# juansgomez87/consensus-entropy

Measured on AMD Instinct MI355X. Metric: pool items scored+ranked/sec (M=16,C=4) at 1/2/4/8 GPUs; % HBM roofline, higher is better.
Workload: dtype f64; 1 GPU; configs[3] large-ensemble pool: 100000000 items x 16 members x 4 classes fp32, [N,M,C] layout=NMC, q=10, sharded over 1 GPU(s); n_items=100000000, members=16, classes=4, q=10, input_dtype=f32, layout=NMC, items_per_gpu=100000000

## Files before the change

### consensus-entropy_amd/csrc/ce_launch_stream.hip

```cpp
#include <atomic>

#include "ce_dispatch.hpp"
#include "ce_stream.hpp"
#include "ce_wide_stream.hpp"

using namespace ce;

static inline StreamArgs stream_args(const CommArgs& a, int G, int64_t base_idx) {
    StreamArgs s;
    s.p = a.p;
    s.N = a.N;
    s.M = a.M;
    s.sN = a.sN;
    s.sM = a.sM;
    s.sC = a.sC;
    s.dM = (double)a.M;
    s.invM = 1.0 / (double)a.M;
    s.pow2 = (a.M & (a.M - 1)) == 0;
    s.base_idx = base_idx;
    s.nlists = G;
    s.per_wave = 0;
    s.excl = nullptr;
    s.ctr = nullptr;
    s.oval = nullptr;
    s.oidx = nullptr;
    s.ocand = nullptr;
    s.extra = nullptr;
    s.vote = nullptr;
    s.vote_heavy = 0;
    s.seed = nullptr;
    s.claim = nullptr;
    s.claim_from = 0;
    return s;
}

static inline void stream_grid(StreamArgs& s, int grid) {
    const int64_t W = (int64_t)grid * 4;
    s.per_wave = (cdiv(s.N, W) + 63) / 64 * 64;
}

template <class Src, class F>
static inline void with_batching(int M, F&& f) {
    if constexpr (Src::kDT == kF64 || Src::kC > 4) {
        (void)M;
        f(std::integral_constant<int, 4>(), std::integral_constant<int, 2>());
    } else {
        if (M <= 4) f(std::integral_constant<int, 4>(), std::integral_constant<int, 4>());
        else f(std::integral_constant<int, 8>(), std::integral_constant<int, 2>());
    }
}


template <int UNR, class F>
static inline void with_unr(int unr, F&& f) {
    if (unr == UNR) f(std::integral_constant<int, UNR>());
    else f(std::integral_constant<int, 1>());
}

static int launch_stream_impl(const CommArgs& a, int G, int q, int64_t base_idx, WsLists w, hipStream_t st,
                              const uint32_t* excl, const FoldOut* fold);

#ifndef CE_STREAM_CLAIM_PERMILLE
#define CE_STREAM_CLAIM_PERMILLE 150
#endif
#ifndef CE_STREAM_CLAIM_MIN_ROUNDS
#define CE_STREAM_CLAIM_MIN_ROUNDS 300
#endif
static std::atomic<int64_t> g_claim_permille{-1}, g_claim_min_rounds{-1}, g_claim_from_last{0};
extern "C" void ce_debug_stream_claims(int64_t permille, int64_t min_rounds) {
    g_claim_permille = permille;
    g_claim_min_rounds = min_rounds;
}
extern "C" int64_t ce_debug_stream_claim_from() { return g_claim_from_last; }

static inline int64_t claim_from(int64_t N, int grid) {
    int64_t permille = g_claim_permille, min_rounds = g_claim_min_rounds;
    if (permille < 0) permille = CE_STREAM_CLAIM_PERMILLE;
    if (min_rounds < 0) min_rounds = CE_STREAM_CLAIM_MIN_ROUNDS;
    if (permille > 1000) permille = 1000;
    const int64_t rounds = cdiv(N, 64) / ((int64_t)grid * 4);
    if (rounds < min_rounds || permille == 0) return 0;
    const int64_t r = rounds - cdiv(rounds * permille, 1000);
    return r < 4 ? 4 : r;
}

#ifndef CE_NMC_AUX
#define CE_NMC_AUX 2
#endif

constexpr int64_t kWideHeavyBytes = 16384;

bool launch_stream(const CommArgs& a, int G, int q, int64_t base_idx, WsLists w, hipStream_t st,
                   const uint32_t* excl) {
    return launch_stream_impl(a, G, q, base_idx, w, st, excl, nullptr) != 0;
}

Stage1 launch_stream_fold(const CommArgs& a, int G, int q, int64_t base_idx, WsLists w, hipStream_t st,
                          const uint32_t* excl, FoldOut out) {
    return static_cast<Stage1>(launch_stream_impl(a, G, q, base_idx, w, st, excl, &out));
}

static int launch_stream_impl(const CommArgs& a, int G, int q, int64_t base_idx, WsLists w, hipStream_t st,
                              const uint32_t* excl, const FoldOut* fold) {
    note_kernel("%s", "");
    if (q > kStreamMaxQ || a.N == 0) return 0;
    StreamArgs sa = stream_args(a, G, base_idx);
    sa.excl = excl;
    if (fold) {
        sa.ctr = w.ctr;
        sa.oval = fold->oval;
        sa.oidx = fold->oidx;
        sa.ocand = fold->ocand;
        sa.extra = fold->extra;
    }
    const int folded = fold ? 2 : 1;
    const int eb = elem_bytes(a.dt);
    const int64_t R = (int64_t)a.M * a.C * eb;
    const bool dense_nmc = a.sC == 1 && a.sM == a.C && a.sN == (int64_t)a.M * a.C && (uintptr_t)a.p % 16 == 0;
#define CE_NMC(MATCH_, DT_, C_, S_, AUX_, MNC_)                                                             \
    if (a.dt == DT_ && a.C == C_ && (MATCH_)) {                                                           \
                   \
        constexpr int RING_ = S_ == 16 ? 2 : 1;                                                           \
        auto kern = k_stream_nmc<DT_, C_, S_, AUX_, MNC_, RING_>;                                         \
        const int grid = resident_grid(kern, 0, G);                                                       \
        note_kernel("ce::k_stream_nmc<%d, %d, %d, %d, %s, %d>", DT_, C_, S_, AUX_, MNC_ ? "true" : "false", \
                    RING_);                                                                               \
        stream_grid(sa, grid);                                                                            \
        g_claim_from_last = 0;                                                                            \
        if (fold && !MNC_ && RING_ == 2 && DT_ == kF32 && C_ == 4 && CE_STREAM_CLAIM_K > 0) {             \
            sa.claim_from = claim_from(a.N, grid);                    \
            sa.claim = sa.claim_from > 0 ? w.ctr + kWsClaimSlot : nullptr;                                \
            g_claim_from_last = sa.claim_from;                                                            \
        }                                                                                                 \
        hipLaunchKernelGGL(kern, dim3(grid), dim3(256), 0, st, sa, q, w.c);                               \
        return folded;                                                                                    \
    }
    if (dense_nmc && (R == 256 || R == 512)) {
#define CE_S(DT_, C_, S_) CE_NMC(R == 16 * S_, DT_, C_, S_, CE_NMC_AUX, false)
        CE_S(kF32, 4, 16) CE_S(kF32, 4, 32) CE_S(kBF16, 4, 16) CE_S(kBF16, 4, 32) CE_S(kF64, 4, 32)
        CE_S(kF32, 8, 16) CE_S(kF32, 8, 32)
#undef CE_S
    }
    const bool dense_mnc = a.sC == 1 && a.sN == a.C && a.C * eb == 16 && (a.sM * eb) % 16 == 0 &&
                           (uintptr_t)a.p % 16 == 0 && a.M >= 4;
    if (dense_mnc) {
#define CE_SM(DT_, C_, M_) CE_NMC(a.M == M_, DT_, C_, M_, 2, true)
        CE_SM(kF32, 4, 4) CE_SM(kF32, 4, 8) CE_SM(kF32, 4, 16) CE_SM(kF32, 4, 20) CE_SM(kF32, 4, 32)
        CE_SM(kF64, 2, 8) CE_SM(kF64, 2, 16) CE_SM(kBF16, 8, 16)
#undef CE_SM
    }
#undef CE_NMC
    int rc = with_committee(a, [&](auto src) {
        using S = decltype(src);
        with_batching<S>(a.M, [&](auto unr, auto ipl) {
            auto kern = k_stream_direct<S, decltype(ipl)::value, decltype(unr)::value>;
            note_kernel("ce::k_stream_direct<ce::CommitteeSrc<%d, %d, %s>, %d, %d>", S::kDT, S::kC,
                        S::kVec ? "true" : "false", decltype(ipl)::value, decltype(unr)::value);
            const int grid = resident_grid(kern, 0, G);
            stream_grid(sa, grid);
            hipLaunchKernelGGL(kern, dim3(grid), dim3(256), 0, st, src, sa, q, w.c);
        });
    });
    if (rc == CE_OK) return folded;
    if (a.C > kWideMaxC) return 0;
    const WideArgs wa = wide_args(a);
    const PwPlan pl = pw_plan(a.C);
    const size_t lds = wide_lds_bytes(a.C);
    int rc_excl = CE_OK;
    bool wide_folded = fold != nullptr;
    rc = with_wide_v(a, [&](auto dt, auto npl, auto vec) {
        constexpr int DT = decltype(dt)::value, NPL = decltype(npl)::value;
        if constexpr (decltype(vec)::value) {
            constexpr int KCH = NPL / ChunkT<DT>::CPC > 0 ? NPL / ChunkT<DT>::CPC : 1;
            constexpr int UNR = KCH >= 4 ? 1 : 4 / KCH;
            const int unr = a.M % UNR == 0 ? UNR : 1;
            auto go = [&](auto kern, int nb, int per_cu, StreamArgs s) {
                note_kernel("ce::k_stream_wide2<%d, %d, %d, %d>", DT, KCH, unr, nb);
                const int grid = std::min(resident_grid(kern, lds, G), per_cu * device_cus());
                stream_grid(s, grid);
                hipLaunchKernelGGL(kern, dim3(grid), dim3(256), lds, st, wa, pl, s, q, w.c);
            };
            bool voted = false;
            if constexpr (KCH <= 2)
                voted = R >= kWideHeavyBytes && fold != nullptr && fold->wide_ws != nullptr &&
                        a.N >= kWideSeedMinItems && CE_WIDE_PREFILTER;
            if (voted) {
                if constexpr (KCH <= 2) {
                    const WideSeedWs sw = wide_seed_carve(fold->wide_ws);
                    const int ns = (int)wide_nsamples(a.N);
                    with_unr<UNR>(unr, [&](auto u) {
                        hipLaunchKernelGGL((k_wide_seed<DT, KCH, decltype(u)::value>), dim3((unsigned)cdiv(ns, 4)),
                                           dim3(256), lds, st, wa, pl, sa.base_idx, sa.excl, sw.samp, sw.sapx);
                    });
                    hipLaunchKernelGGL(k_wide_seed_pick<kWideVoteSamples>, dim3(1), dim3(1024), 0, st, sw.samp, sw.sapx, ns, q,
                                       fold->extra, sw.seed, sw.vote);
                    StreamArgs sh = sa, so = sa;
                    sh.vote = so.vote = sw.vote;
                    sh.seed = so.seed = sw.seed;
                    sh.vote_heavy = 1;
                    so.vote_heavy = 0;
                    with_unr<UNR>(unr, [&](auto u) {
                        go(k_stream_wide2<DT, KCH, decltype(u)::value, 8>, 8, 1, sh);
                        go(k_stream_wide2<DT, KCH, decltype(u)::value, 2>, 2, 1 << 20, so);
                    });
                    note_kernel("ce::k_stream_wide2<%d, %d, %d, 8>|ce::k_stream_wide2<%d, %d, %d, 2>", DT, KCH, unr,
                                DT, KCH, unr);
                }
            } else {
                with_unr<UNR>(unr, [&](auto u) { go(k_stream_wide2<DT, KCH, decltype(u)::value, 2>, 2, 1 << 20, sa); });
            }
        } else {
            if (sa.excl) {
                rc_excl = CE_EUNSUPPORTED;
                return;
            }
            sa.ctr = nullptr;
            wide_folded = false;
            auto kern = k_stream_wide<DT, NPL, false>;
            note_kernel("ce::k_stream_wide<%d, %d, false>", DT, NPL);
            const int grid = resident_grid(kern, lds, G);
            stream_grid(sa, grid);
            hipLaunchKernelGGL(kern, dim3(grid), dim3(256), lds, st, wa, pl, sa, q, w.c);
        }
    });
    if (rc != CE_OK || rc_excl != CE_OK) return 0;
    return wide_folded ? 2 : 1;
}

#ifdef CE_STREAM_STAMPS
extern "C" int ce_debug_stream_stamps(uint64_t* host, int waves) {
    if (waves < 0 || waves > kStampWaves) return -1;
    return hipMemcpyFromSymbol(host, HIP_SYMBOL(g_stream_stamps), (size_t)waves * kStampCols * sizeof(uint64_t)) ==
                   hipSuccess
               ? 0
               : -1;
}
extern "C" int ce_debug_stream_stamp_cols() { return kStampCols; }
#endif
```

### consensus-entropy_amd/csrc/ce_stream.hpp

```cpp
#pragma once
#include "ce_device.hpp"
#include "ce_merge.hpp"
#include "ce_topq.hpp"
#include "ce_wave.hpp"
#include "ce_ws.hpp"

namespace ce {

template <int S>
struct ItemTile {
    uint32_t u[S * 4];

    template <int AUX>
    __device__ __forceinline__ static void issue(const char* base, int64_t t0, int n_valid, char* lds) {
        const int lane = threadIdx.x & 63;
#pragma unroll
        for (int k = 0; k < S; ++k) {
            const int p = k * 64 + lane;
            const int r = p / S, s = p % S;
            const int rs = r < n_valid ? r : n_valid - 1;
            const int m = s ^ (r & 15);
            const char* src = base + (t0 + rs) * (int64_t)(16 * S) + 16 * m;
            __builtin_amdgcn_global_load_lds(
                (const void*)src, (void __attribute__((address_space(3)))*)(lds + k * 1024), 16, 0, AUX);
        }
    }

    template <int AUX>
    __device__ __forceinline__ static void issue_mnc(const char* base, int64_t t0, int n_valid, int64_t sMb,
                                                     char* lds) {
        const int lane = threadIdx.x & 63;
        const int64_t it = t0 + (lane < n_valid ? lane : n_valid - 1);
#pragma unroll
        for (int k = 0; k < S; ++k) {
            const char* src = base + (int64_t)k * sMb + it * 16;
            __builtin_amdgcn_global_load_lds(
                (const void*)src, (void __attribute__((address_space(3)))*)(lds + k * 1024), 16, 0, AUX);
        }
    }

    __device__ __forceinline__ void read_mnc(const char* lds) {
        const int lane = threadIdx.x & 63;
        typedef unsigned int u32x4 __attribute__((ext_vector_type(4)));
#pragma unroll
        for (int m = 0; m < S; ++m) {
            const u32x4 v = *reinterpret_cast<const u32x4*>(lds + m * 1024 + lane * 16);
            u[4 * m + 0] = v.x;
            u[4 * m + 1] = v.y;
            u[4 * m + 2] = v.z;
            u[4 * m + 3] = v.w;
        }
    }

    __device__ __forceinline__ void read(const char* lds) {
        const int lane = threadIdx.x & 63;
        typedef unsigned int u32x4 __attribute__((ext_vector_type(4)));
#pragma unroll
        for (int m = 0; m < S; ++m) {
            const u32x4 v = *reinterpret_cast<const u32x4*>(lds + lane * 16 * S + 16 * (m ^ (lane & 15)));
            u[4 * m + 0] = v.x;
            u[4 * m + 1] = v.y;
            u[4 * m + 2] = v.z;
            u[4 * m + 3] = v.w;
        }
    }

    template <int DT>
    __device__ __forceinline__ double elem(int e) const {
        if constexpr (DT == kF32)
            return (double)__uint_as_float(u[e]);
        else if constexpr (DT == kF64)
            return __longlong_as_double((long long)(((uint64_t)u[2 * e + 1] << 32) | u[2 * e]));
        else
            return bf16_to_f64((u[e >> 1] >> (16 * (e & 1))) & 0xffffu);
    }

    template <int DT, int C>
    __device__ __forceinline__ void mean(double dM, double invM, bool pow2, double (&mean)[C]) const {
        constexpr int EB = DT == kF64 ? 8 : (DT == kF32 ? 4 : 2);
        constexpr int M = 16 * S / (C * EB);
        static_assert(M * C * EB == 16 * S, "tile row must hold whole members");
        double acc[C];
#pragma unroll
        for (int c = 0; c < C; ++c) acc[c] = 0.0;
#pragma unroll
        for (int m = 0; m < M; ++m)
#pragma unroll
            for (int c = 0; c < C; ++c) acc[c] += elem<DT>(m * C + c);
#pragma unroll
        for (int c = 0; c < C; ++c) mean[c] = div_members(acc[c], dM, invM, pow2);
    }
};

template <int S, int RING = 1>
struct StreamSmemNMC {
    char tile[4][RING][64 * 16 * S];
    WaveLists lists;
};

struct StreamArgs {
    const void* p;
    int64_t N;
    int M;
    int64_t sN, sM, sC;
    double dM, invM;
    bool pow2;
    int64_t base_idx;
    int64_t per_wave;
    const uint32_t* excl;
    int nlists;
    uint32_t* ctr;
    double* oval;
    int64_t* oidx;
    Cand* ocand;
    const Cand* extra;
    const uint32_t* vote;
    int vote_heavy;
    const Cand* seed;
    uint32_t* claim;
    int64_t claim_from;
};

template <int DT, int C, int S>
__device__ __forceinline__ void score_tile(const ItemTile<S>& t, const StreamArgs& a, int64_t t0, int64_t hi,
                                           RegTopQ& tq) {
    double mean[C];
    t.template mean<DT, C>(a.dM, a.invM, a.pow2, mean);
    const double h = entropy_row<C>(mean);
    const int64_t i = t0 + (threadIdx.x & 63);
    bool ok = i < hi;
    if (a.excl) ok = ok && !excluded(a.excl, i < hi ? i : hi - 1);
    tq.offer(order_key(h), i + a.base_idx, ok);
}

#ifndef CE_STREAM_CLAIM_K
#define CE_STREAM_CLAIM_K 8
#endif

#ifdef CE_STREAM_STAMPS
constexpr int kStampWaves = 4096, kStampSamples = 12, kStampCols = 6 + 2 * kStampSamples;
__device__ uint64_t g_stream_stamps[kStampWaves][kStampCols];
struct StreamStampSmem {
    uint64_t s[4][2 * kStampSamples];
};
#endif

template <int DT, int C, int S, int AUX, bool MNC = false, int RING = 1>
__global__ __launch_bounds__(256) void k_stream_nmc(StreamArgs a, int q, Cand* __restrict__ wc) {
    static_assert(RING == 1 || RING == 2, "one or two tiles per wave");
    CE_DASSERT((int)gridDim.x <= a.nlists && q >= 1 && q <= kStreamMaxQ);
    __shared__ __attribute__((aligned(16))) StreamSmemNMC<S, RING> sm;
    const int w = threadIdx.x >> 6, lane = threadIdx.x & 63;
    RegTopQ tq;
    tq.init(q);
    const char* base = static_cast<const char*>(a.p);
    constexpr int EB = DT == kF64 ? 8 : (DT == kF32 ? 4 : 2);
    const int64_t sMb = a.sM * EB;
    auto issue = [&](int64_t t, int nv, int slot) {
        char* lds = sm.tile[w][slot];
        if constexpr (MNC) ItemTile<S>::template issue_mnc<AUX>(base, t, nv, sMb, lds);
        else ItemTile<S>::template issue<AUX>(base, t, nv, lds);
    };
    ItemTile<S> t;
#ifdef CE_STREAM_STAMPS
    __shared__ StreamStampSmem stamps;
    const int64_t gw = (int64_t)blockIdx.x * 4 + w;
    const int64_t st_waves = (int64_t)gridDim.x * 4;
    const int64_t st_every = max<int64_t>(1, (((a.N + 63) / 64 + st_waves - 1) / st_waves + kStampSamples - 1) / kStampSamples);
    int64_t st_it = 0;
    int st_n = 0;
    uint64_t st_landed = 0;
    uint64_t st_first = 0;
#define CE_SSAMPLE(tile_)                                            \
    {                                                                \
        if (st_it % st_every == 0 && st_n < kStampSamples) {         \
            if (lane == 0) {                                         \
                stamps.s[w][2 * st_n] = wall_clock64();              \
                stamps.s[w][2 * st_n + 1] = (uint64_t)(tile_);       \
            }                                                        \
            ++st_n;                                                  \
        }                                                            \
        ++st_it;                                                     \
    }
#define CE_SLANDED(last_) \
    if (last_) st_landed = wall_clock64();
#define CE_SSTAMP(col_) \
    if (lane == 0 && gw < kStampWaves) g_stream_stamps[gw][col_] = wall_clock64();
#define CE_SFIRST() st_first = wall_clock64();
#else
#define CE_SSAMPLE(tile_)
#define CE_SLANDED(last_)
#define CE_SSTAMP(col_)
#define CE_SFIRST()
#endif
    bool claims = false;
    if constexpr (!MNC && RING == 2 && CE_STREAM_CLAIM_K > 0) claims = a.claim != nullptr;
    if (claims) {
        if constexpr (!MNC && RING == 2 && CE_STREAM_CLAIM_K > 0) {
            constexpr int K = CE_STREAM_CLAIM_K;
            static_assert(K == 2 || K == 4 || K == 8, "an even number of tiles per unit");
            const int wu = __builtin_amdgcn_readfirstlane(w);
            const int64_t nt = (a.N + 63) >> 6;
            const int64_t W = (int64_t)gridDim.x * 4, g = (int64_t)blockIdx.x * 4 + wu, R = a.claim_from;
            const int64_t T0 = R * W;
            CE_DASSERT(R >= 4);
            int64_t ta = min<int64_t>(g, nt), tb = min<int64_t>(g + W, nt);
            CE_SFIRST()
            if (ta < nt) issue(ta * 64, (int)min<int64_t>(64, a.N - ta * 64), 0);
            if (tb < nt) issue(tb * 64, (int)min<int64_t>(64, a.N - tb * 64), 1);
            stage_log_table();
            int64_t js = 2, ibase = nt;
            int isub = 0, slot = 0;
            bool claimed = false, dead = false;
            uint32_t c = 0;
            bool claimed_prev = false;
            while (ta < nt) {
                if (tb < nt) {
                    if (claimed_prev) asm volatile("s_waitcnt vmcnt(%0)" ::"n"(S + 1) : "memory");
                    else asm volatile("s_waitcnt vmcnt(%0)" ::"n"(S) : "memory");
                } else {
                    asm volatile("s_waitcnt vmcnt(0)" ::: "memory");
                }
                CE_SLANDED(tb >= nt)
                t.read(sm.tile[w][slot]);
                asm volatile("s_waitcnt lgkmcnt(0)" ::: "memory");
                __builtin_amdgcn_sched_barrier(0);
                int64_t tc;
                bool want;
                if (js < R) {
                    tc = g + js * W;
                    want = js == R - 2;
                    ++js;
                } else {
                    if (!claimed || ++isub == K) {
                        claimed = true;
                        isub = 0;
                        ibase = dead ? nt : T0 + (int64_t)K * (int64_t)(uint32_t)__builtin_amdgcn_readfirstlane((int)c);
                    }
                    tc = ibase + isub;
                    want = isub == 0;
                }
                if (tc >= nt) {
                    tc = nt;
                    dead = true;
                }
                claimed_prev = want && !dead;
                if (claimed_prev && lane == 0)
                    c = __builtin_amdgcn_atomic_inc32(a.claim, 0xffffffffu, __ATOMIC_RELAXED, "agent");
                if (tc < nt) issue(tc * 64, (int)min<int64_t>(64, a.N - tc * 64), slot);
                slot ^= 1;
                CE_SSAMPLE(ta)
                score_tile<DT, C, S>(t, a, ta * 64, a.N, tq);
                ta = tb;
                tb = tc;
            }
        }
    } else {
        stage_log_table();
        int64_t lo, hi, step;
        if constexpr (!MNC) {
            const int64_t W = (int64_t)gridDim.x * 4;
            lo = ((int64_t)blockIdx.x * 4 + w) * 64;
            hi = a.N;
            step = W * 64;
        } else {
            const int64_t blo = (int64_t)blockIdx.x * 4 * a.per_wave;
            hi = blo + 4 * a.per_wave < a.N ? blo + 4 * a.per_wave : a.N;
            lo = blo + 64 * w;
            step = 256;
        }
        if (lo > hi) lo = hi;
        CE_SFIRST()
#pragma unroll
        for (int r = 0; r < RING; ++r)
            if (lo + r * step < hi) issue(lo + r * step, (int)min<int64_t>(64, hi - lo - r * step), r);
        int slot = 0;
        for (int64_t t0 = lo; t0 < hi; t0 += step) {
            if constexpr (RING == 2) {
                if (t0 + step < hi) asm volatile("s_waitcnt vmcnt(%0)" ::"n"(S) : "memory");
                else asm volatile("s_waitcnt vmcnt(0)" ::: "memory");
            } else {
                asm volatile("s_waitcnt vmcnt(0)" ::: "memory");
            }
            CE_SLANDED(!(t0 + step < hi))
            const char* lds = sm.tile[w][slot];
            if constexpr (MNC) t.read_mnc(lds);
            else t.read(lds);
            asm volatile("s_waitcnt lgkmcnt(0)" ::: "memory");
            __builtin_amdgcn_sched_barrier(0);
            const int64_t t1 = t0 + RING * step;
            if (t1 < hi) issue(t1, (int)min<int64_t>(64, hi - t1), slot);
            slot = RING == 1 ? 0 : slot ^ 1;
            CE_SSAMPLE(t0 / 64)
            score_tile<DT, C, S>(t, a, t0, hi, tq);
        }
    }
#ifdef CE_STREAM_STAMPS
    if (lane == 0 && gw < kStampWaves) {
        uint64_t* row = g_stream_stamps[gw];
        row[0] = st_first;
        row[1] = st_landed;
        row[3] = 0;
        row[4] = (uint64_t)st_it;
        row[5] = (uint64_t)st_n;
        for (int k = 0; k < 2 * kStampSamples; ++k) row[6 + k] = k < 2 * st_n ? stamps.s[w][k] : 0;
    }
#endif
    block_merge_write<4>(tq, sm.lists, q, wc + (int64_t)blockIdx.x * q, a.nlists, nullptr, nullptr, 4, a.ctr != nullptr);
    CE_SSTAMP(2)
    if (a.ctr) fold_merge<4>(a.ctr, a.oval, a.oidx, a.ocand, q, wc, sm.lists, a.extra, claims ? a.claim : nullptr);
    CE_SSTAMP(3)
#undef CE_SSAMPLE
#undef CE_SLANDED
#undef CE_SSTAMP
#undef CE_SFIRST
}

template <class Src, int IPL, int UNR>
__device__ __forceinline__ void stream_direct_range(const Src& src, int64_t lo, int64_t hi, int64_t rel, int q,
                                                    RegTopQ& tq, const uint32_t* excl = nullptr) {
    const int lane = threadIdx.x & 63;
    for (int64_t t0 = lo; t0 < hi; t0 += 64 * IPL) {
        uint64_t k[IPL];
        int64_t items[IPL];
#pragma unroll
        for (int u = 0; u < IPL; ++u) {
            const int64_t i = t0 + 64 * u + lane;
            items[u] = i < hi ? i : hi - 1;
        }
        src.template keys<UNR, IPL>(items, k);
#pragma unroll
        for (int u = 0; u < IPL; ++u) {
            const int64_t i = t0 + 64 * u + lane;
            bool ok = i < hi;
            if (excl) ok = ok && !excluded(excl, items[u]);
            tq.offer(k[u], i + rel, ok);
        }
    }
}

template <class Src, int IPL, int UNR>
__global__ __launch_bounds__(256) void k_stream_direct(Src src, StreamArgs a, int q, Cand* __restrict__ wc) {
    stage_log_table();
    CE_DASSERT((int)gridDim.x <= a.nlists && q >= 1 && q <= kStreamMaxQ);
    __shared__ WaveLists sm;
    const int w = threadIdx.x >> 6;
    const int64_t gw = (int64_t)blockIdx.x * 4 + w;
    int64_t lo = gw * a.per_wave;
    int64_t hi = lo + a.per_wave;
    if (hi > a.N) hi = a.N;
    if (lo > hi) lo = hi;
    RegTopQ tq;
    tq.init(q);
    stream_direct_range<Src, IPL, UNR>(src, lo, hi, a.base_idx, q, tq, a.excl);
    block_merge_write<4>(tq, sm, q, wc + (int64_t)blockIdx.x * q, a.nlists, nullptr, nullptr, 4, a.ctr != nullptr);
    if (a.ctr) fold_merge<4>(a.ctr, a.oval, a.oidx, a.ocand, q, wc, sm, a.extra);
}

template <class Src, int IPL, int UNR, int WAVES>
__global__ __launch_bounds__(64 * WAVES) void k_stream_seg(Src src, const int64_t* __restrict__ offsets, int64_t n,
                                                            int64_t base_idx, int q, int bpu,
                                                            double* __restrict__ oval, int64_t* __restrict__ oidx,
                                                            Cand* __restrict__ wc, const uint32_t* __restrict__ excl) {
    stage_log_table();
    __shared__ WaveListsT<WAVES> sm;
    __shared__ uint64_t fk_s[4 * WAVES];
    __shared__ int64_t fi_s[4 * WAVES];
    const int w = threadIdx.x >> 6, nw = blockDim.x >> 6, lane = threadIdx.x & 63;
    const int u = blockIdx.x / bpu, part = blockIdx.x % bpu;
    const int64_t s0 = offsets ? offsets[u] : 0, s1 = offsets ? offsets[u + 1] : n;
    const int64_t len = s1 > s0 ? s1 - s0 : 0;
    constexpr int64_t kIt = 64 * IPL;
    const int64_t its = (len + kIt - 1) / kIt;
    const int64_t its_b = (its + bpu - 1) / bpu;
    const int64_t its_w = (its_b + nw - 1) / nw;
    int64_t lo = s0 + ((int64_t)part * its_b + (int64_t)w * its_w) * kIt;
    int64_t hi_b = s0 + ((int64_t)part + 1) * its_b * kIt;
    if (hi_b > s1) hi_b = s1;
    int64_t hi = lo + its_w * kIt < hi_b ? lo + its_w * kIt : hi_b;
    if (lo > hi) lo = hi;
    const int64_t rel = (offsets ? 0 : base_idx) - s0;
    uint64_t k0[IPL];
    int64_t it0[IPL];
    bool ok0[IPL];
#pragma unroll
    for (int v = 0; v < IPL; ++v) {
        const int64_t i = lo + 64 * v + lane;
        it0[v] = i < hi ? i : hi - 1;
        ok0[v] = false;
        k0[v] = 0;
    }
    if (lo < hi) {
        src.template keys<UNR, IPL>(it0, k0);
#pragma unroll
        for (int v = 0; v < IPL; ++v) {
            ok0[v] = lo + 64 * v + lane < hi;
            if (excl) ok0[v] = ok0[v] && !excluded(excl, it0[v]);
        }
    }
    uint64_t bk = 0;
    int64_t bi = INT64_MAX;
#pragma unroll
    for (int v = 0; v < IPL; ++v)
        if (ok0[v] && better(k0[v], lo + 64 * v + lane + rel, bk, bi)) {
            bk = k0[v];
            bi = lo + 64 * v + lane + rel;
        }
    row_best16(bk, bi);
    if ((lane & 15) == 0) {
        fk_s[w * 4 + (lane >> 4)] = bk;
        fi_s[w * 4 + (lane >> 4)] = bi;
    }
    __syncthreads();
    uint64_t fk = 0;
    int64_t fi = INT64_MAX;
    const int nb = 4 * nw;
    if (q <= nb) {
        bool hit = false;
        uint64_t vk = 0;
        int64_t vi = INT64_MAX;
        if (lane < nb) {
            vk = fk_s[lane];
            vi = fi_s[lane];
            int rank = 0;
            for (int v = 0; v < nb; ++v) rank += better(fk_s[v], fi_s[v], vk, vi);
            hit = vi != INT64_MAX && rank == q - 1;
        }
        const uint64_t m = __ballot(hit);
        if (m) {
            const int sl = __builtin_ctzll(m);
            fk = readlane64(vk, sl);
            fi = (int64_t)readlane64((uint64_t)vi, sl) + 1;
        }
    }
    RegTopQ tq;
    tq.init(q, fk, fi);
#pragma unroll
    for (int v = 0; v < IPL; ++v) tq.offer(k0[v], lo + 64 * v + lane + rel, ok0[v]);
    if (lo + kIt < hi) stream_direct_range<Src, IPL, UNR>(src, lo + kIt, hi, rel, q, tq, excl);
    if (bpu == 1) {
        const int64_t slot = (int64_t)u * q;
        block_merge_write<WAVES>(tq, sm, q, nullptr, 0, oval + slot, oidx + slot, nw);
    } else {
        block_merge_write<WAVES>(tq, sm, q, wc + (int64_t)blockIdx.x * q, 0, nullptr, nullptr, nw);
    }
}

}
```

### consensus-entropy_amd/csrc/ce_wave.hpp

```cpp
#pragma once
#include "ce_device.hpp"
#include "ce_topq.hpp"

namespace ce {

__device__ __forceinline__ uint64_t readlane64(uint64_t v, int l) {
    const uint32_t lo = (uint32_t)__builtin_amdgcn_readlane((int)(uint32_t)v, l);
    const uint32_t hi = (uint32_t)__builtin_amdgcn_readlane((int)(uint32_t)(v >> 32), l);
    return ((uint64_t)hi << 32) | lo;
}

__device__ __forceinline__ void shfl_cand(uint64_t& k, int64_t& i, int src) {
    const int a = src << 2;
    const uint32_t k0 = (uint32_t)__builtin_amdgcn_ds_bpermute(a, (int)(uint32_t)k);
    const uint32_t k1 = (uint32_t)__builtin_amdgcn_ds_bpermute(a, (int)(uint32_t)(k >> 32));
    const uint32_t i0 = (uint32_t)__builtin_amdgcn_ds_bpermute(a, (int)(uint32_t)(uint64_t)i);
    const uint32_t i1 = (uint32_t)__builtin_amdgcn_ds_bpermute(a, (int)(uint32_t)((uint64_t)i >> 32));
    k = ((uint64_t)k1 << 32) | k0;
    i = (int64_t)(((uint64_t)i1 << 32) | i0);
}

template <int J>
__device__ __forceinline__ uint32_t xor_lane(uint32_t v) {
    if constexpr (J == 1) {
        return (uint32_t)__builtin_amdgcn_update_dpp(0, (int)v, 0xB1, 0xF, 0xF, false);
    } else if constexpr (J == 2) {
        return (uint32_t)__builtin_amdgcn_update_dpp(0, (int)v, 0x4E, 0xF, 0xF, false);
    } else if constexpr (J == 4) {
        const int t = __builtin_amdgcn_update_dpp(0, (int)v, 0x141, 0xF, 0xF, false);
        return (uint32_t)__builtin_amdgcn_update_dpp(0, t, 0x1B, 0xF, 0xF, false);
    } else if constexpr (J == 8) {
        return (uint32_t)__builtin_amdgcn_update_dpp(0, (int)v, 0x128, 0xF, 0xF, false);
    } else if constexpr (J == 16) {
        const auto p = __builtin_amdgcn_permlane16_swap(v, v, false, false);
        return (threadIdx.x & 16) ? p[0] : p[1];
    } else {
        static_assert(J == 32, "lane exchange distance");
        const auto p = __builtin_amdgcn_permlane32_swap(v, v, false, false);
        return (threadIdx.x & 32) ? p[0] : p[1];
    }
}

__device__ __forceinline__ uint64_t lane_above(uint64_t v) {
    const uint32_t lo = (uint32_t)__builtin_amdgcn_update_dpp(0, (int)(uint32_t)v, 0x138, 0xF, 0xF, false);
    const uint32_t hi = (uint32_t)__builtin_amdgcn_update_dpp(0, (int)(uint32_t)(v >> 32), 0x138, 0xF, 0xF, false);
    return ((uint64_t)hi << 32) | lo;
}

template <int J>
__device__ __forceinline__ void xor_cand(uint64_t& k, int64_t& i) {
    const uint32_t k0 = xor_lane<J>((uint32_t)k), k1 = xor_lane<J>((uint32_t)(k >> 32));
    const uint32_t i0 = xor_lane<J>((uint32_t)(uint64_t)i), i1 = xor_lane<J>((uint32_t)((uint64_t)i >> 32));
    k = ((uint64_t)k1 << 32) | k0;
    i = (int64_t)(((uint64_t)i1 << 32) | i0);
}

template <int J>
__device__ __forceinline__ void cx_stage(uint64_t& k, int64_t& i, bool desc) {
    const int lane = threadIdx.x & 63;
    uint64_t pk = k;
    int64_t pi = i;
    xor_cand<J>(pk, pi);
    const bool lower = (lane & J) == 0;
    const bool pb = better(pk, pi, k, i);
    const bool take = (lower == desc) ? pb : !pb;
    if (take) {
        k = pk;
        i = pi;
    }
}

template <int S, int J>
__device__ __forceinline__ void sort_stages(uint64_t& k, int64_t& i) {
    cx_stage<J>(k, i, ((threadIdx.x & 63) & S) == 0);
    if constexpr (J > 1) sort_stages<S, J / 2>(k, i);
}

template <int S>
__device__ __forceinline__ void sort_levels(uint64_t& k, int64_t& i) {
    sort_stages<S, S / 2>(k, i);
    if constexpr (S < 64) sort_levels<S * 2>(k, i);
}

template <int J>
__device__ __forceinline__ void best_stages(uint64_t& k, int64_t& i) {
    uint64_t pk = k;
    int64_t pi = i;
    xor_cand<J>(pk, pi);
    if (better(pk, pi, k, i)) {
        k = pk;
        i = pi;
    }
    if constexpr (J < 32) best_stages<J * 2>(k, i);
}
__device__ __forceinline__ void wave_best64(uint64_t& k, int64_t& i) { best_stages<1>(k, i); }

__device__ __forceinline__ void row_best16(uint64_t& k, int64_t& i) {
    uint64_t pk;
    int64_t pi;
#define CE_RB(J)                          \
    pk = k;                               \
    pi = i;                               \
    xor_cand<J>(pk, pi);                  \
    if (better(pk, pi, k, i)) {           \
        k = pk;                           \
        i = pi;                           \
    }
    CE_RB(1) CE_RB(2) CE_RB(4) CE_RB(8)
#undef CE_RB
}

__device__ __forceinline__ void wave_sort64(uint64_t& k, int64_t& i) { sort_levels<2>(k, i); }

__device__ __forceinline__ void wave_merge64(uint64_t& k, int64_t& i, uint64_t bk, int64_t bi) {
    const int lane = threadIdx.x & 63;
    shfl_cand(bk, bi, 63 - lane);
    if (better(bk, bi, k, i)) {
        k = bk;
        i = bi;
    }
    sort_stages<64, 32>(k, i);
}

struct NoHook {
    __device__ __forceinline__ void operator()() const {}
};

__device__ __forceinline__ bool excluded(const uint32_t* b, int64_t i) { return (b[i >> 5] >> (i & 31)) & 1u; }

struct RegTopQ {
    uint64_t k;
    int64_t i;
    uint64_t tk;
    int64_t ti;
    uint64_t fk;
    int64_t fi;
    int q;

    __device__ __forceinline__ void init(int q_, uint64_t fk_ = 0, int64_t fi_ = INT64_MAX) {
        k = 0;
        i = INT64_MAX;
        tk = fk = fk_;
        ti = fi = fi_;
        q = q_;
    }

    __device__ __forceinline__ void refresh() {
        const uint64_t sk = readlane64(k, q - 1);
        const int64_t si = (int64_t)readlane64((uint64_t)i, q - 1);
        const bool s_better = better(sk, si, fk, fi);
        tk = s_better ? sk : fk;
        ti = s_better ? si : fi;
    }

    __device__ __forceinline__ bool empty() const { return readlane64((uint64_t)i, 0) == (uint64_t)INT64_MAX; }

    __device__ __forceinline__ void insert(uint64_t ck, int64_t ci) {
        const int lane = threadIdx.x & 63;
        const uint64_t below = __ballot(better(ck, ci, k, i));
        const int p = __builtin_ctzll(below);
        const uint64_t uk = lane_above(k);
        const int64_t ui = (int64_t)lane_above((uint64_t)i);
        if (lane > p) {
            k = uk;
            i = ui;
        } else if (lane == p) {
            k = ck;
            i = ci;
        }
    }

    __device__ __forceinline__ void offer(uint64_t ck, int64_t ci, bool valid) {
        const bool pass = valid && better(ck, ci, tk, ti);
        uint64_t mask = __ballot(pass);
        if (mask == 0) return;
        if (__popcll(mask) <= 8) {
            do {
                const int s = __builtin_ctzll(mask);
                mask &= mask - 1;
                const uint64_t sk = readlane64(ck, s);
                const int64_t si = (int64_t)readlane64((uint64_t)ci, s);
                if (better(sk, si, tk, ti)) {
                    insert(sk, si);
                    refresh();
                }
            } while (mask);
        } else {
            uint64_t bk = pass ? ck : 0ull;
            int64_t bi = pass ? ci : INT64_MAX;
            wave_sort64(bk, bi);
            if (empty()) {
                k = bk;
                i = bi;
            } else {
                wave_merge64(k, i, bk, bi);
            }
            refresh();
        }
    }
};


template <int WAVES>
struct WaveListsT {
    uint64_t key[WAVES][64];
    int64_t idx[WAVES][64];
};
using WaveLists = WaveListsT<4>;

__device__ __forceinline__ void store_cand_wt(Cand* p, uint64_t k, int64_t i) {
    __hip_atomic_store(&p->key, k, __ATOMIC_RELAXED, __HIP_MEMORY_SCOPE_AGENT);
    __hip_atomic_store(&p->idx, i, __ATOMIC_RELAXED, __HIP_MEMORY_SCOPE_AGENT);
}
__device__ __forceinline__ Cand load_cand_wt(const Cand* p) {
    Cand c;
    c.key = __hip_atomic_load(&p->key, __ATOMIC_RELAXED, __HIP_MEMORY_SCOPE_AGENT);
    c.idx = __hip_atomic_load(&p->idx, __ATOMIC_RELAXED, __HIP_MEMORY_SCOPE_AGENT);
    return c;
}
__device__ __forceinline__ bool arrive_last(uint32_t* ctr, uint32_t n, int* lds_ticket) {
    asm volatile("s_waitcnt vmcnt(0)" ::: "memory");
    __syncthreads();
    if (threadIdx.x == 0) *lds_ticket = (int)__builtin_amdgcn_atomic_inc32(ctr, n - 1, __ATOMIC_RELAXED, "agent");
    __syncthreads();
    const int t = *lds_ticket;
    CE_DASSERT(t >= 0 && t < (int)n);
    return t == (int)n - 1;
}

template <int WAVES>
__device__ inline void block_merge_write(const RegTopQ& tq, WaveListsT<WAVES>& L, int q, Cand* wc, int nlists,
                                         double* oval = nullptr, int64_t* oidx = nullptr, int nw = WAVES,
                                         bool wt = false) {
    const int w = threadIdx.x >> 6, lane = threadIdx.x & 63;
    for (int64_t s = (int64_t)blockIdx.x + gridDim.x; s < nlists; s += gridDim.x)
        for (int r = threadIdx.x; r < q; r += blockDim.x) wc[(s - blockIdx.x) * q + r] = Cand{0ull, -1};
    uint64_t k = tq.k;
    int64_t i = tq.i;
    for (int s = 1; s < WAVES && s < nw; s <<= 1) {
        if ((w & (2 * s - 1)) == s) {
            L.key[w][lane] = k;
            L.idx[w][lane] = i;
        }
        __syncthreads();
        if ((w & (2 * s - 1)) == 0) {
            const uint64_t bk = L.key[w + s][lane];
            const int64_t bi = L.idx[w + s][lane];
            if (readlane64((uint64_t)bi, 0) != (uint64_t)INT64_MAX) {
                if (readlane64((uint64_t)i, 0) == (uint64_t)INT64_MAX) {
                    k = bk;
                    i = bi;
                } else {
                    wave_merge64(k, i, bk, bi);
                }
            }
        }
    }
    if (w == 0 && lane < q) {
        const bool ok = i != INT64_MAX;
        if (oval) {
            oval[lane] = ok ? key_to_val(k) : __longlong_as_double(0x7ff8000000000000ll);
            oidx[lane] = ok ? i : -1;
        } else if (wt) {
            store_cand_wt(wc + lane, ok ? k : 0ull, ok ? i : -1);
        } else {
            wc[lane] = Cand{ok ? k : 0ull, ok ? i : -1};
        }
    }
}

}
```

Before: 27.94 billion items/s.

## Defer claim atomic readback via pinned VGPR and scalarize exclusion bitmap loads

Replaces the compiler-generated atomic_inc for work claiming with inline asm that issues a returning global atomic into a fixed VGPR and reads the result later, waiting on vmcnt only if the value has not yet landed. The aim is to keep the claim latency from serializing with the tile loads. It also lowers the claim minimum-rounds threshold so dynamic claiming starts on smaller inputs. Exclusion-bitmap checks become two uniform scalar loads per tile instead of per-lane vector loads. Hardcoding v200 outside the compiler's register allocation and relying on a sentinel value is fragile, and debug counters are added under the stamps build.

```diff
diff --git a/consensus-entropy_amd/csrc/ce_launch_stream.hip b/consensus-entropy_amd/csrc/ce_launch_stream.hip
--- a/consensus-entropy_amd/csrc/ce_launch_stream.hip
+++ b/consensus-entropy_amd/csrc/ce_launch_stream.hip
@@ -64,7 +64,7 @@
 #define CE_STREAM_CLAIM_PERMILLE 150
 #endif
 #ifndef CE_STREAM_CLAIM_MIN_ROUNDS
-#define CE_STREAM_CLAIM_MIN_ROUNDS 300
+#define CE_STREAM_CLAIM_MIN_ROUNDS 150
 #endif
 static std::atomic<int64_t> g_claim_permille{-1}, g_claim_min_rounds{-1}, g_claim_from_last{0};
 extern "C" void ce_debug_stream_claims(int64_t permille, int64_t min_rounds) {
@@ -236,4 +236,11 @@
                : -1;
 }
 extern "C" int ce_debug_stream_stamp_cols() { return kStampCols; }
-#endif
+extern "C" int ce_debug_stream_claim_counts(uint64_t* host) {
+    static_assert(sizeof(unsigned long long) == sizeof(uint64_t), "");
+    const unsigned long long zero[2] = {0, 0};
+    if (hipDeviceSynchronize() != hipSuccess) return -1;
+    if (hipMemcpyFromSymbol(host, HIP_SYMBOL(g_stream_claim_counts), sizeof(zero)) != hipSuccess) return -1;
+    return hipMemcpyToSymbol(HIP_SYMBOL(g_stream_claim_counts), zero, sizeof(zero)) == hipSuccess ? 0 : -1;
+}
+#endif
diff --git a/consensus-entropy_amd/csrc/ce_stream.hpp b/consensus-entropy_amd/csrc/ce_stream.hpp
--- a/consensus-entropy_amd/csrc/ce_stream.hpp
+++ b/consensus-entropy_amd/csrc/ce_stream.hpp
@@ -129,12 +129,36 @@
     const double h = entropy_row<C>(mean);
     const int64_t i = t0 + (threadIdx.x & 63);
     bool ok = i < hi;
-    if (a.excl) ok = ok && !excluded(a.excl, i < hi ? i : hi - 1);
+    if (a.excl) ok = ok && !excluded_tile(a.excl, t0, a.N);
     tq.offer(order_key(h), i + a.base_idx, ok);
 }
 
 #ifndef CE_STREAM_CLAIM_K
 #define CE_STREAM_CLAIM_K 8
+#endif
+
+#define CE_CLAIM_VGPR "v200"
+__device__ __forceinline__ void claim_issue(uint32_t* word) {
+    asm volatile("v_mov_b32 " CE_CLAIM_VGPR ", -1\n\t"
+                 "global_atomic_add " CE_CLAIM_VGPR ", %0, %1, %2 sc0"
+                 :
+                 : "v"(0u), "v"(1u), "s"(word)
+                 : CE_CLAIM_VGPR, "memory");
+}
+__device__ __forceinline__ uint32_t claim_result(bool& late) {
+    uint32_t v;
+    asm volatile("v_readfirstlane_b32 %0, " CE_CLAIM_VGPR "\n\ts_nop 4" : "=s"(v) : : CE_CLAIM_VGPR, "memory");
+    late = v == 0xffffffffu;
+    if (late)
+        asm volatile("s_waitcnt vmcnt(0)\n\tv_readfirstlane_b32 %0, " CE_CLAIM_VGPR "\n\ts_nop 4"
+                     : "=s"(v)
+                     :
+                     : CE_CLAIM_VGPR, "memory");
+    return v;
+}
+
+#ifdef CE_STREAM_STAMPS
+__device__ unsigned long long g_stream_claim_counts[2];
 #endif
 
 #ifdef CE_STREAM_STAMPS
@@ -187,7 +211,12 @@
 #define CE_SSTAMP(col_) \
     if (lane == 0 && gw < kStampWaves) g_stream_stamps[gw][col_] = wall_clock64();
 #define CE_SFIRST() st_first = wall_clock64();
+    unsigned st_claims = 0, st_late = 0;
+#define CE_SCLAIM(late_) \
+    ++st_claims;         \
+    st_late += (late_) ? 1u : 0u;
 #else
+#define CE_SCLAIM(late_) (void)(late_);
 #define CE_SSAMPLE(tile_)
 #define CE_SLANDED(last_)
 #define CE_SSTAMP(col_)
@@ -212,7 +241,6 @@
             int64_t js = 2, ibase = nt;
             int isub = 0, slot = 0;
             bool claimed = false, dead = false;
-            uint32_t c = 0;
             bool claimed_prev = false;
             while (ta < nt) {
                 if (tb < nt) {
@@ -235,7 +263,12 @@
                     if (!claimed || ++isub == K) {
                         claimed = true;
                         isub = 0;
-                        ibase = dead ? nt : T0 + (int64_t)K * (int64_t)(uint32_t)__builtin_amdgcn_readfirstlane((int)c);
+                        ibase = nt;
+                        if (!dead) {
+                            bool late;
+                            ibase = T0 + (int64_t)K * (int64_t)claim_result(late);
+                            CE_SCLAIM(late)
+                        }
                     }
                     tc = ibase + isub;
                     want = isub == 0;
@@ -245,8 +278,7 @@
                     dead = true;
                 }
                 claimed_prev = want && !dead;
-                if (claimed_prev && lane == 0)
-                    c = __builtin_amdgcn_atomic_inc32(a.claim, 0xffffffffu, __ATOMIC_RELAXED, "agent");
+                if (claimed_prev && lane == 0) claim_issue(a.claim);
                 if (tc < nt) issue(tc * 64, (int)min<int64_t>(64, a.N - tc * 64), slot);
                 slot ^= 1;
                 CE_SSAMPLE(ta)
@@ -305,6 +337,10 @@
         row[5] = (uint64_t)st_n;
         for (int k = 0; k < 2 * kStampSamples; ++k) row[6 + k] = k < 2 * st_n ? stamps.s[w][k] : 0;
     }
+    if (lane == 0 && st_claims) {
+        atomicAdd(&g_stream_claim_counts[0], (unsigned long long)st_claims);
+        atomicAdd(&g_stream_claim_counts[1], (unsigned long long)st_late);
+    }
 #endif
     block_merge_write<4>(tq, sm.lists, q, wc + (int64_t)blockIdx.x * q, a.nlists, nullptr, nullptr, 4, a.ctr != nullptr);
     CE_SSTAMP(2)
@@ -314,6 +350,7 @@
 #undef CE_SLANDED
 #undef CE_SSTAMP
 #undef CE_SFIRST
+#undef CE_SCLAIM
 }
 
 template <class Src, int IPL, int UNR>
diff --git a/consensus-entropy_amd/csrc/ce_wave.hpp b/consensus-entropy_amd/csrc/ce_wave.hpp
--- a/consensus-entropy_amd/csrc/ce_wave.hpp
+++ b/consensus-entropy_amd/csrc/ce_wave.hpp
@@ -127,6 +127,20 @@
 };
 
 __device__ __forceinline__ bool excluded(const uint32_t* b, int64_t i) { return (b[i >> 5] >> (i & 31)) & 1u; }
+
+__device__ __forceinline__ bool excluded_tile(const uint32_t* b, int64_t t0, int64_t n) {
+    typedef const __attribute__((address_space(4))) uint32_t* cptr;
+    const int lane = threadIdx.x & 63;
+    const uint64_t wv = (uint64_t)t0 >> 5;
+    const uint64_t w0 = ((uint64_t)(uint32_t)__builtin_amdgcn_readfirstlane((int)(uint32_t)(wv >> 32)) << 32) |
+                        (uint32_t)__builtin_amdgcn_readfirstlane((int)(uint32_t)wv);
+    const uint64_t words = (uint64_t)(n + 31) >> 5;
+    CE_DASSERT((t0 & 63) == 0 && w0 < words);
+    const cptr c = (cptr)(uintptr_t)b;
+    const uint32_t x0 = c[w0];
+    const uint32_t x1 = w0 + 1 < words ? c[w0 + 1] : 0u;
+    return (((lane & 32) ? x1 : x0) >> (lane & 31)) & 1u;
+}
 
 struct RegTopQ {
     uint64_t k;
```

New measurement: 27.93 billion items/s. No clear change (-0.0%).
